# colmap/pycolmap

Measured on AMD Instinct MI355X. Metric: descriptor-pair distances/sec (exhaustive SIFT match: dot + top-2 + ratio + cross-check), higher is better.
Workload: dtype u8 descriptors, int8 MFMA / int32 accumulate; 1 GPU; 500 images x 4096 descriptors, exhaustive match + ratio test + cross-check (BASELINE.json configs[1] at N=1); pairs_total=124750, pairs_per_rank=124750, kernel=auto, matches_rank0=1865611

## Files before the change

### pycolmap_amd/csrc/match_mfma.hip

```cpp
#include <cstdlib>

#include "amc_internal.h"
#include "scan_accept.h"

namespace amc {

typedef int i32x4 __attribute__((ext_vector_type(4)));
typedef __attribute__((address_space(1))) const void gvoid_t;
typedef __attribute__((address_space(3))) void lvoid_t;

constexpr int kBN = 128;
constexpr int kYS = kBN / 32;
constexpr int kUR = 128;
constexpr int kSPB = kUR / 32;
constexpr int kChunkBytes = kBN * kDim;
constexpr int kW = kSegsPerItem;
constexpr int kWGPerCU = 2;
constexpr int kXT = kSegRows / 16;
constexpr int kKeyShift = 7, kKeyCarried = 127;

constexpr int kNB = 4;
constexpr int kOffRs = 0;
constexpr int kOffQ = kOffRs + kNB * kBN * 4;
constexpr int kOffB = kOffQ + 16;
constexpr int kLdsBytes = kOffB + kNB * kChunkBytes;
static_assert(kRowPad % kBN == 0, "a chunk divides the row padding: every chunk that holds a row lies inside the padded image");
static_assert(kUR == 128 && kSPB == 4 && kBN == kUR, "a lane quarter's rows of a block are one 32-row tile; the loop body is one block, which is one chunk");
static_assert(kRowPad % kSegRows == 0 && kSegRows % 32 == 0, "segments tile the padded rows");
static_assert((kNB & (kNB - 1)) == 0, "the ring position is taken modulo kNB with a mask");
static_assert(kWGPerCU * (kLdsBytes + 16) <= 160 * 1024, "LDS of one CU holds two workgroups (and their copy-part slots)");
static_assert(kW == 4, "one wave of a workgroup per SIMD");
static_assert(sizeof(SegDesc) == 64, "a descriptor is 16 dwords: one per lane of a quarter wave");

enum : int { kDXprep = 0, kDXrs = 2, kDOut = 4, kDList = 6, kDYprep = 8, kDYrs = 10, kDCnt = 12, kDAccword = 13,
             kDYrows = 14 };

__device__ __forceinline__ void mfma_first(i32x4& d, const i32x4& a, const i32x4& b, const i32x4& c) {
    asm volatile("v_mfma_i32_16x16x64_i8 %0, %1, %2, %3" : "=&v"(d) : "v"(a), "v"(b), "v"(c));
}
__device__ __forceinline__ void mfma_acc(i32x4& d, const i32x4& a, const i32x4& b) {
    asm volatile("v_mfma_i32_16x16x64_i8 %0, %1, %2, %0" : "+v"(d) : "v"(a), "v"(b));
}

struct YFrag {
    i32x4 f[2][2];
    i32x4 ci[2];
};

#ifdef AMC_SCAN_STAMPS
constexpr int kStampMaxWG = 1024;
__device__ uint32_t g_scan_stamps[2 * kStampMaxWG * kSegsPerItem * 8];
#define AMC_STAMP() ((uint32_t)__builtin_amdgcn_s_memtime())
#endif

__device__ __noinline__ __attribute__((used)) void copy_part(const uint4* __restrict__ src, uint4* __restrict__ dst,
                                                             unsigned long long b, unsigned long long e, int tid,
                                                             int nthreads) {
    __builtin_assume(tid >= 0 && tid < 1024 && nthreads >= 256 && nthreads <= 512);
    unsigned long long i = b + (unsigned long long)tid;
    const unsigned long long st = (unsigned long long)nthreads;
    for (; i + 3 * st < e; i += 4 * st) {
        const uint4 v0 = src[i], v1 = src[i + st], v2 = src[i + 2 * st], v3 = src[i + 3 * st];
        dst[i] = v0; dst[i + st] = v1; dst[i + 2 * st] = v2; dst[i + 3 * st] = v3;
    }
    for (; i < e; i += st) dst[i] = src[i];
}

template <int MODE>
__global__ __launch_bounds__(64 * kW) __attribute__((amdgpu_waves_per_eu(kWGPerCU, kWGPerCU)))
void match_mfma_kernel(const SegDesc* __restrict__ segs, const uint32_t* __restrict__ nitems_p,
                       uint32_t* __restrict__ queue_head, uint32_t* __restrict__ accmask,
                       const ScanAccept* __restrict__ accept, CopyJob job, uint32_t* __restrict__ copy_head) {
    static_assert(kChunkBytes / 1024 == kW * kYS, "a chunk splits into 1 KiB DMA pieces, one per wave and step");
    static_assert(kBN * 4 == 512, "a chunk's rs128 block is half a wave's DMA");
    __shared__ __attribute__((aligned(16))) char smem[kLdsBytes];

    const int tid = threadIdx.x;
    const int lane = tid & 63;
    const int wid = __builtin_amdgcn_readfirstlane(tid >> 6);
    const int l15 = lane & 15, lq = lane >> 4;
    volatile uint32_t* s_q = reinterpret_cast<volatile uint32_t*>(smem + kOffQ);
    if constexpr (MODE == 0) {
        if (job.parts) {
            __shared__ uint32_t s_part;
            if (tid == 0) s_part = atomicAdd(copy_head, 1u);
            __syncthreads();
            const uint32_t part = s_part;
            if (part < job.parts)
                copy_part(static_cast<const uint4*>(job.src), static_cast<uint4*>(job.dst), job.n16 * part / job.parts,
                          job.n16 * (part + 1) / job.parts, tid, 64 * kW);
        }
    }
    const uint32_t nitems = *nitems_p;
    const ScanAccept sa = *accept;

    auto load_desc = [&](uint32_t q) -> int {
        int v = 0;
        if (q < nitems && lane < 16) v = reinterpret_cast<const int*>(segs + (size_t)q * kSegsPerItem + wid)[lane];
        return v;
    };
    auto dword = [&](int dv, int f) -> int { return __builtin_amdgcn_readlane(dv, f); };
    auto dptr = [&](int dv, int f) -> const char* {
        const uint64_t lo = (uint32_t)__builtin_amdgcn_readlane(dv, f);
        const uint64_t hi = (uint32_t)__builtin_amdgcn_readlane(dv, f + 1);
        return reinterpret_cast<const char*>(lo | (hi << 32));
    };

    constexpr int kPW = kChunkBytes / 1024 / kW;
    auto stage_piece = [&](const char* yprep, int c, int buf, int ps) __attribute__((always_inline)) {
        const int piece = ps * kW + wid;
        __builtin_amdgcn_global_load_lds((gvoid_t*)(yprep + (size_t)c * kChunkBytes + piece * 1024 + lane * 16),
                                         (lvoid_t*)(smem + kOffB + buf * kChunkBytes + piece * 1024), 16, 0, 0);
    };
    auto stage_rs = [&](const char* yrs, int c, int buf) __attribute__((always_inline)) {
        if (wid == 0 && lane < kBN / 4)
            __builtin_amdgcn_global_load_lds((gvoid_t*)(yrs + (size_t)c * kBN * 4 + lane * 16),
                                             (lvoid_t*)(smem + kOffRs + buf * kBN * 4), 16, 0, 0);
    };
    auto stage = [&](const char* yprep, const char* yrs, int c, int buf) __attribute__((always_inline)) {
#pragma unroll
        for (int ps = 0; ps < kPW; ++ps) stage_piece(yprep, c, buf, ps);
        stage_rs(yrs, c, buf);
    };
    auto stage_head = [&](int dv) __attribute__((always_inline)) {
        const char* yprep = dptr(dv, kDYprep);
        const char* yrs = dptr(dv, kDYrs);
        const int yrows = dword(dv, kDYrows);
        stage(yprep, yrs, 0, 0);
#pragma unroll
        for (int c = 1; c < kNB - 1; ++c)
            if (yrows > c * kBN) stage(yprep, yrs, c, c);
    };

    const int yrow_lane = (kUR / 4) * (l15 >> 2) + (l15 & 3);
    const int ysw_lane = arena_swizzle(yrow_lane);
    const int yoff0 = kOffB + yrow_lane * kDim + ((lq ^ ysw_lane) * 16);
    const int yoff1 = kOffB + yrow_lane * kDim + (((4 + lq) ^ ysw_lane) * 16);
    const int coff = kOffRs + (kUR / 4) * lq * 4;
    auto load_y_part = [&](YFrag& y, int buf, int ys, int part) __attribute__((always_inline)) {
        const int ub = (ys / kSPB) * kUR, sp = ys % kSPB;
        if (part < 2) {
            const int so = buf * kBN * 4 + (ub + 8 * sp) * 4;
            y.ci[part] = *reinterpret_cast<const i32x4*>(smem + (coff + so) + 16 * part);
        } else {
            const int tt = (part - 2) >> 1, s = (part - 2) & 1;
            const int so = buf * kChunkBytes + (ub + 8 * sp) * kDim;
            y.f[tt][s] = *reinterpret_cast<const i32x4*>(smem + ((s ? yoff1 : yoff0) + so) + tt * 4 * kDim);
        }
    };
    auto load_y = [&](YFrag& y, int buf, int ys) __attribute__((always_inline)) {
#pragma unroll
        for (int part = 0; part < 6; ++part) load_y_part(y, buf, ys, part);
    };

    i32x4 xf[kXT][2];
    int best[kXT], sec[kXT], btile[kXT], xterm[kXT], part[kXT];
    auto load_x = [&](int dv) __attribute__((always_inline)) {
        const int cnt = dword(dv, kDCnt);
        const char* xprep = dptr(dv, kDXprep);
        const int* xrs = reinterpret_cast<const int*>(dptr(dv, kDXrs));
#pragma unroll
        for (int xt = 0; xt < kXT; ++xt) {
            const int kl = xt * 16 + l15;
            int row;
            if (MODE == 0) {
                row = kl;
            } else {
                const uint32_t* list = reinterpret_cast<const uint32_t*>(dptr(dv, kDList));
                row = cnt > 0 ? (int)list[min(kl, cnt - 1)] : 0;
            }
            const char* rp = xprep + (size_t)row * kDim;
            const int sw = arena_swizzle(row);
#pragma unroll
            for (int s = 0; s < 2; ++s) xf[xt][s] = *reinterpret_cast<const i32x4*>(rp + (((4 * s + lq) ^ sw) * 16));
            xterm[xt] = xrs[row] - (1 << 21);
            best[xt] = ((-xterm[xt]) << kKeyShift) | kKeyCarried;
            sec[xt] = best[xt];
            btile[xt] = -1;
        }
    };

#ifdef AMC_SCAN_STAMPS
    uint32_t st_a = 0, st_first = 0, st_end = 0, st_sum[5] = {0, 0, 0, 0, 0};
    bool st_prev = false, st_prev_active = false;
    uint32_t* const st_slot = g_scan_stamps + ((size_t)(MODE * kStampMaxWG + min((int)blockIdx.x, kStampMaxWG - 1)) * kW + wid) * 8;
#endif
    if (tid == 0) *s_q = atomicAdd(queue_head, 1u);
    __syncthreads();
    uint32_t q = *s_q;
    int dv = load_desc(q);
    if (q < nitems) {
        stage_head(dv);
        if (dword(dv, kDCnt) > 0) load_x(dv);
    }
    __syncthreads();

    while (q < nitems) {
        const char* yprep = dptr(dv, kDYprep);
        const char* yrs = dptr(dv, kDYrs);
        const int nchunks = (dword(dv, kDYrows) + kBN - 1) / kBN;
        const bool active = dword(dv, kDCnt) > 0;
        if (tid == 0) *s_q = atomicAdd(queue_head, 1u);

        i32x4 acc[2][2];
        auto insert = [&](int xt, int code) __attribute__((always_inline)) {
            asm volatile(
                "v_lshl_or_b32 %2, %2, 7, %3\n\t"
                "v_med3_i32 %1, %0, %1, %2\n\t"
                "v_max_i32 %0, %0, %2"
                : "+v"(best[xt]), "+v"(sec[xt]), "+v"(part[xt])
                : "s"(code));
        };
        auto flush = [&](int sb) __attribute__((always_inline)) {
#pragma unroll
            for (int xt = 0; xt < kXT; ++xt) {
                const int c = best[xt] & 127;
                btile[xt] = c != kKeyCarried ? sb * 64 + (126 - c) : btile[xt];
                best[xt] |= kKeyCarried;
            }
        };
        auto phase = [&](i32x4 (&an)[2], const YFrag& y, int xtn, const i32x4 (&ac)[2], int xtc, int sp, int gb)
                         __attribute__((always_inline)) {
            mfma_first(an[0], y.f[0][0], xf[xtn][0], y.ci[0]);
            mfma_first(an[1], y.f[1][0], xf[xtn][0], y.ci[1]);
            __builtin_amdgcn_sched_barrier(0);
            if (xtc == 0 ? sp == 0 : sp == kSPB - 1) {
                insert((xtc + kXT - 1) % kXT, 126 - ((xtc == 0 ? gb - 1 : gb) & 63));
                if (xtc == 0 && gb != 0 && (gb & 63) == 0) flush((gb >> 6) - 1);
                __builtin_amdgcn_sched_barrier(0);
            }
            mfma_acc(an[0], y.f[0][1], xf[xtn][1]);
            mfma_acc(an[1], y.f[1][1], xf[xtn][1]);
            __builtin_amdgcn_sched_barrier(0);
            int t0, t1;
            if (sp == 0)
                asm volatile(
                    "v_max3_i32 %0, %3, %4, %5\n\t"
                    "v_max3_i32 %1, %6, %7, %8\n\t"
                    "v_max3_i32 %0, %0, %9, %10\n\t"
                    "v_max_i32 %2, %0, %1"
                    : "=&v"(t0), "=&v"(t1), "=&v"(part[xtc])
                    : "v"(ac[0][0]), "v"(ac[0][1]), "v"(ac[0][2]), "v"(ac[0][3]), "v"(ac[1][0]), "v"(ac[1][1]),
                      "v"(ac[1][2]), "v"(ac[1][3]));
            else
                asm volatile(
                    "v_max3_i32 %0, %3, %4, %5\n\t"
                    "v_max3_i32 %1, %6, %7, %8\n\t"
                    "v_max3_i32 %0, %0, %9, %10\n\t"
                    "v_max3_i32 %2, %0, %1, %2"
                    : "=&v"(t0), "=&v"(t1), "+v"(part[xtc])
                    : "v"(ac[0][0]), "v"(ac[0][1]), "v"(ac[0][2]), "v"(ac[0][3]), "v"(ac[1][0]), "v"(ac[1][1]),
                      "v"(ac[1][2]), "v"(ac[1][3]));
            __builtin_amdgcn_sched_barrier(0);
        };

        YFrag y0, y1;
        asm volatile("s_waitcnt vmcnt(0)" ::: "memory");
        __syncthreads();
        const uint32_t qn = *s_q;
        const int dvn = load_desc(qn);
#ifdef AMC_SCAN_STAMPS
        {
            const uint32_t now = AMC_STAMP();
            if (st_prev) {
                st_sum[0] += st_a;
                st_sum[1] += now - st_end;
                st_sum[2] += now - st_first;
                st_sum[3] += 1;
                st_sum[4] += st_prev_active ? 1 : 0;
                if (lane == 0) {
#pragma unroll
                    for (int k = 0; k < 5; ++k) st_slot[k] = st_sum[k];
                }
            }
            st_a = 0;
            st_first = now;
        }
#endif
        if (active) {
            load_y(y0, 0, 0);
            mfma_first(acc[0][0], y0.f[0][0], xf[0][0], y0.ci[0]);
            mfma_first(acc[0][1], y0.f[1][0], xf[0][0], y0.ci[1]);
            mfma_acc(acc[0][0], y0.f[0][1], xf[0][1]);
            mfma_acc(acc[0][1], y0.f[1][1], xf[0][1]);
            part[kXT - 1] = -(1 << 24);
            __builtin_amdgcn_sched_barrier(0);
        }
        auto step = [&](YFrag& yc, YFrag& yn, int c, int cb, int nb, int ys) __attribute__((always_inline)) {
            const int sp = ys;
            const bool lastt = ys == kYS - 1;
            const bool cross = lastt && (c + 1 < nchunks);
            const bool fetch = c + kNB - 1 < nchunks;
            static_assert(kPW == kYS, "one DMA piece per wave and step");
            if (fetch) {
                const int fb = (cb + kNB - 1) & (kNB - 1);
                stage_piece(yprep, c + kNB - 1, fb, ys);
                if (ys == 0) stage_rs(yrs, c + kNB - 1, fb);
            }
            if (cross) {
#ifdef AMC_SCAN_STAMPS
                const uint32_t st_t = AMC_STAMP();
#endif
                static_assert(kNB == 4, "the counted waits below are written out for three chunks ahead");
                if (fetch) {
                    if (wid == 0) asm volatile("s_waitcnt vmcnt(%0)" ::"n"(2 * kPW + 2) : "memory");
                    else asm volatile("s_waitcnt vmcnt(%0)" ::"n"(2 * kPW) : "memory");
                } else if (c + 2 < nchunks) {
                    if (wid == 0) asm volatile("s_waitcnt vmcnt(%0)" ::"n"(kPW + 1) : "memory");
                    else asm volatile("s_waitcnt vmcnt(%0)" ::"n"(kPW) : "memory");
                } else {
                    asm volatile("s_waitcnt vmcnt(0)" ::: "memory");
                }
                asm volatile("s_barrier" ::: "memory");
#ifdef AMC_SCAN_STAMPS
                st_a += AMC_STAMP() - st_t;
#endif
            }
            if (active) {
                const int nbuf = cross ? nb : cb;
                const int nys = lastt ? (cross ? 0 : ys) : ys + 1;
                const int gb = c;
#pragma unroll
                for (int xt = 0; xt < kXT; ++xt) {
                    if (xt + 1 < kXT)
                        phase(acc[(xt + 1) & 1], yc, xt + 1, acc[xt & 1], xt, sp, gb);
                    else
                        phase(acc[0], yn, 0, acc[xt & 1], xt, sp, gb);
                    if (xt < 6) {
                        load_y_part(yn, nbuf, nys, xt);
                        __builtin_amdgcn_sched_barrier(0);
                    }
                }
            }
        };
#pragma unroll 1
        for (int c = 0; c < nchunks; ++c) {
            const int cb = c & (kNB - 1), nb = (c + 1) & (kNB - 1);
            step(y0, y1, c, cb, nb, 0);
            step(y1, y0, c, cb, nb, 1);
            step(y0, y1, c, cb, nb, 2);
            step(y1, y0, c, cb, nb, 3);
        }
        if (active) {
            const int lastb = nchunks - 1;
            insert(kXT - 1, 126 - (lastb & 63));
            flush(lastb >> 6);
#pragma unroll
            for (int xt = 0; xt < kXT; ++xt) {
                best[xt] >>= kKeyShift;
                sec[xt] >>= kKeyShift;
            }
        }
        __syncthreads();
#ifdef AMC_SCAN_STAMPS
        st_end = AMC_STAMP();
        st_prev = true;
        st_prev_active = active;
#endif

        int eb[kXT], es[kXT], et[kXT], ex[kXT];
#pragma unroll
        for (int xt = 0; xt < kXT; ++xt) {
            asm volatile("v_mov_b32 %0, %1" : "=v"(eb[xt]) : "v"(best[xt]));
            asm volatile("v_mov_b32 %0, %1" : "=v"(es[xt]) : "v"(sec[xt]));
            asm volatile("v_mov_b32 %0, %1" : "=v"(et[xt]) : "v"(btile[xt]));
            ex[xt] = xterm[xt];
        }
        if (qn < nitems) {
            stage_head(dvn);
            if (dword(dvn, kDCnt) > 0) load_x(dvn);
        }
        if (active) {
            const int cnt = dword(dv, kDCnt);
            uint32_t bits_lo = 0;
#pragma unroll
            for (int xt = 0; xt < kXT; ++xt) {
                const int kl = xt * 16 + l15;
                int b = eb[xt], s = es[xt], t = et[xt] < 0 ? -1 : et[xt] * kSPB + lq;
#pragma unroll
                for (int m = 16; m <= 32; m <<= 1) {
                    const int ob = __shfl_xor(b, m);
                    const int os = __shfl_xor(s, m);
                    const int ot = __shfl_xor(t, m);
                    const bool ow = (ob > b) || (ob == b && (unsigned)ot < (unsigned)t);
                    s = max(max(s, os), ow ? b : ob);
                    t = ow ? ot : t;
                    b = ow ? ob : b;
                }
                bool acc_bit = false;
                const bool live = lq == 0 && kl < cnt;
                Top2 o;
                o.best_v = (uint32_t)(b + ex[xt]);
                o.best_idx = o.best_v ? (uint32_t)t : 0xFFFFFFFFu;
                o.second_v = (uint32_t)(s + ex[xt]);
                o.pad = 0;
                if (MODE == 0) acc_bit = live && scan_may_accept(sa, o.best_v, o.second_v);
                const uint32_t bits = MODE == 0 ? (uint32_t)__ballot(acc_bit) : 0u;
                if (live && (MODE == 1 || bits != 0)) {
                    Top2* out = reinterpret_cast<Top2*>(const_cast<char*>(dptr(dv, kDOut)));
                    int row = kl;
                    if (MODE == 1) row = (int)reinterpret_cast<const uint32_t*>(dptr(dv, kDList))[kl];
                    out[row] = o;
                }
                if (MODE == 0) {
                    if (xt & 1) {
                        const uint32_t word = bits_lo | (bits << 16);
                        if (lane == 0 && word != 0) accmask[(uint32_t)dword(dv, kDAccword) + (xt >> 1)] = word;
                    } else {
                        bits_lo = bits;
                    }
                }
            }
        }
#ifdef AMC_SCAN_STAMPS
        if (qn >= nitems && lane == 0) {
            st_slot[5] = st_a;
            st_slot[6] = AMC_STAMP() - st_first;
            st_slot[7] = 1;
        }
#endif
        q = qn;
        dv = dvn;
    }
}

__device__ __forceinline__ uint32_t pair_segments(int mode, const ImageDev* imgs, const PairDev& p, uint32_t pi,
                                                  const uint32_t* cand_cnt, uint32_t* nrows_out) {
    const uint32_t nx = mode == 0 ? imgs[p.slot1].rows : cand_cnt[pi];
    const uint32_t ny = imgs[mode == 0 ? p.slot2 : p.slot1].rows;
    *nrows_out = nx;
    return ny ? (nx + kSegRows - 1) / kSegRows : 0u;
}

__global__ __launch_bounds__(256) void seg_count_kernel(int mode, const ImageDev* __restrict__ imgs,
                                                        const PairDev* __restrict__ pairs,
                                                        const uint32_t* __restrict__ order,
                                                        const uint32_t* __restrict__ grp_start,
                                                        const uint32_t* __restrict__ cand_cnt,
                                                        uint32_t* __restrict__ seg_base, uint32_t* __restrict__ grp_segs) {
    __shared__ uint32_t wsum[4];
    const uint32_t g = blockIdx.x, tid = threadIdx.x, lane = tid & 63, wid = tid >> 6;
    const uint32_t i0 = grp_start[g], i1 = grp_start[g + 1];
    uint32_t running = 0;
    for (uint32_t base = i0; base < i1; base += 256) {
        const uint32_t i = base + tid;
        uint32_t s = 0, nr;
        if (i < i1) {
            const uint32_t pi = order[i];
            s = pair_segments(mode, imgs, pairs[pi], pi, cand_cnt, &nr);
        }
        uint32_t inc = s;
#pragma unroll
        for (int m = 1; m < 64; m <<= 1) {
            const uint32_t o = __shfl_up(inc, m);
            if (lane >= (uint32_t)m) inc += o;
        }
        if (lane == 63) wsum[wid] = inc;
        __syncthreads();
        uint32_t wbase = 0, total = 0;
        for (uint32_t k = 0; k < 4; ++k) {
            if (k < wid) wbase += wsum[k];
            total += wsum[k];
        }
        if (i < i1) seg_base[i] = running + wbase + inc - s;
        running += total;
        __syncthreads();
    }
    if (tid == 0) grp_segs[g] = running;
}

__global__ __launch_bounds__(1024) void seg_scan_kernel(const uint32_t* __restrict__ grp_segs, uint32_t ngroups,
                                                        uint32_t* __restrict__ grp_item_base,
                                                        uint32_t* __restrict__ nitems_out) {
    __shared__ uint32_t wsum[16];
    const uint32_t tid = threadIdx.x, lane = tid & 63, wid = tid >> 6;
    uint32_t running = 0;
    for (uint32_t base = 0; base < ngroups; base += 1024) {
        const uint32_t g = base + tid;
        const uint32_t s = g < ngroups ? (grp_segs[g] + kSegsPerItem - 1) / kSegsPerItem : 0u;
        uint32_t inc = s;
#pragma unroll
        for (int m = 1; m < 64; m <<= 1) {
            const uint32_t o = __shfl_up(inc, m);
            if (lane >= (uint32_t)m) inc += o;
        }
        if (lane == 63) wsum[wid] = inc;
        __syncthreads();
        uint32_t wbase = 0, total = 0;
        for (uint32_t k = 0; k < 16; ++k) {
            if (k < wid) wbase += wsum[k];
            total += wsum[k];
        }
        if (g < ngroups) grp_item_base[g] = running + wbase + inc - s;
        running += total;
        __syncthreads();
    }
    if (tid == 0) *nitems_out = running;
}

constexpr uint32_t kFillY = 8;
__global__ __launch_bounds__(256) void seg_fill_kernel(int mode, const ImageDev* __restrict__ imgs,
                                                       const PairDev* __restrict__ pairs,
                                                       const uint32_t* __restrict__ order,
                                                       const uint32_t* __restrict__ grp_start,
                                                       const uint32_t* __restrict__ cand_cnt,
                                                       const uint32_t* __restrict__ candbuf,
                                                       const uint32_t* __restrict__ seg_base,
                                                       const uint32_t* __restrict__ grp_segs,
                                                       const uint32_t* __restrict__ grp_item_base,
                                                       Top2* __restrict__ outbuf, SegDesc* __restrict__ segs) {
    const uint32_t g = blockIdx.x, tid = threadIdx.x, lane = tid & 63, wid = blockIdx.y * 4 + (tid >> 6);
    const uint32_t i0 = grp_start[g], i1 = grp_start[g + 1];
    if (i0 >= i1) return;
    const uint32_t total = grp_segs[g];
    if (total == 0) return;
    SegDesc* gs = segs + (size_t)grp_item_base[g] * kSegsPerItem;
    const PairDev p0 = pairs[order[i0]];
    const ImageDev Y = imgs[mode == 0 ? p0.slot2 : p0.slot1];
    for (uint32_t i = i0 + wid; i < i1; i += 4 * kFillY) {
        const uint32_t pi = order[i];
        const PairDev p = pairs[pi];
        uint32_t nx;
        const uint32_t ns = pair_segments(mode, imgs, p, pi, cand_cnt, &nx);
        const ImageDev X = imgs[mode == 0 ? p.slot1 : p.slot2];
        const uint32_t sb = seg_base[i];
        for (uint32_t k = lane; k < ns; k += 64) {
            const uint32_t row0 = k * kSegRows;
            SegDesc d;
            d.yprep = Y.prep;
            d.yrs = Y.rs128;
            d.yrows = Y.rows;
            d.cnt = min(nx - row0, (uint32_t)kSegRows);
            d.pad_ = 0;
            if (mode == 0) {
                d.xprep = X.prep + (size_t)row0 * kDim;
                d.xrs = X.rs128 + row0;
                d.out = outbuf + p.row_off + row0;
                d.list = nullptr;
                d.accword = (uint32_t)((p.row_off + row0) >> 5);
            } else {
                d.xprep = X.prep;
                d.xrs = X.rs128;
                d.out = outbuf + p.col_off;
                d.list = candbuf + p.col_off + row0;
                d.accword = 0;
            }
            gs[sb + k] = d;
        }
    }
    const uint32_t padded = (total + kSegsPerItem - 1) / kSegsPerItem * kSegsPerItem;
    if (blockIdx.y == 0 && tid < padded - total) {
        SegDesc d;
        d.xprep = Y.prep;
        d.xrs = Y.rs128;
        d.out = nullptr;
        d.list = nullptr;
        d.yprep = Y.prep;
        d.yrs = Y.rs128;
        d.cnt = 0;
        d.accword = 0;
        d.yrows = Y.rows;
        d.pad_ = 0;
        gs[total + tid] = d;
    }
}

hipError_t launch_build_segments(int mode, const ImageDev* imgs, const PairDev* pairs, const uint32_t* order,
                                 const uint32_t* grp_start, uint32_t ngroups, const uint32_t* cand_cnt,
                                 const uint32_t* candbuf, Top2* outbuf, uint32_t* seg_base, uint32_t* grp_segs,
                                 uint32_t* grp_item_base, SegDesc* segs, uint32_t* nitems_dev, hipStream_t s) {
    if (ngroups == 0) return memset_async(nitems_dev, 0, sizeof(uint32_t), s);
    hipLaunchKernelGGL(seg_count_kernel, dim3(ngroups), dim3(256), 0, s, mode, imgs, pairs, order, grp_start,
                       cand_cnt, seg_base, grp_segs);
    hipLaunchKernelGGL(seg_scan_kernel, dim3(1), dim3(1024), 0, s, grp_segs, ngroups, grp_item_base, nitems_dev);
    hipLaunchKernelGGL(seg_fill_kernel, dim3(ngroups, kFillY), dim3(256), 0, s, mode, imgs, pairs, order, grp_start,
                       cand_cnt, candbuf, seg_base, grp_segs, grp_item_base, outbuf, segs);
    return hipGetLastError();
}

hipError_t launch_match_mfma(int mode, const SegDesc* segs, const uint32_t* nitems_dev, uint32_t max_items,
                             uint32_t* queue_head, uint32_t* accmask, const ScanAccept* accept_dev, hipStream_t s,
                             const CopyJob& job_in, uint32_t* copy_head) {
    if (max_items == 0) return hipSuccess;
    CopyJob job = (mode == 0 && copy_head) ? job_in : CopyJob();
    hipError_t e = job.parts ? memset_async(copy_head, 0, sizeof(uint32_t), s) : hipSuccess;
    if (e != hipSuccess) return e;
    int dev = 0, cus = 256;
    if ((e = hipGetDevice(&dev)) != hipSuccess) return e;
    if ((e = hipDeviceGetAttribute(&cus, hipDeviceAttributeMultiprocessorCount, dev)) != hipSuccess) return e;
    static const hipError_t occupancy = [] {
        int n0 = 0, n1 = 0;
        hipError_t oe = hipOccupancyMaxActiveBlocksPerMultiprocessor(&n0, match_mfma_kernel<0>, 64 * kW, 0);
        if (oe == hipSuccess) oe = hipOccupancyMaxActiveBlocksPerMultiprocessor(&n1, match_mfma_kernel<1>, 64 * kW, 0);
        if (oe != hipSuccess) return oe;
        return n0 >= kWGPerCU && n1 >= kWGPerCU ? hipSuccess : hipErrorLaunchOutOfResources;
    }();
    if (occupancy != hipSuccess) return occupancy;
    int wgs = kWGPerCU * cus;
    static const int grid_cap = [] {
        const char* e = std::getenv("AMC_SCAN_GRID");
        return e ? std::atoi(e) : 0;
    }();
    if (grid_cap > 0 && grid_cap < wgs) wgs = grid_cap;
    const uint32_t grid = max_items < (uint32_t)wgs ? max_items : (uint32_t)wgs;
    if (job.parts > grid) job.parts = grid;
    if ((e = memset_async(queue_head, 0, sizeof(uint32_t), s)) != hipSuccess) return e;
    if (mode == 0)
        hipLaunchKernelGGL((match_mfma_kernel<0>), dim3(grid), dim3(64 * kW), 0, s, segs, nitems_dev, queue_head,
                           accmask, accept_dev, job, copy_head);
    else
        hipLaunchKernelGGL((match_mfma_kernel<1>), dim3(grid), dim3(64 * kW), 0, s, segs, nitems_dev, queue_head,
                           accmask, accept_dev, job, copy_head);
    return hipGetLastError();
}

}
```

Before: 13580 billion distances/s.

## Split chunk loop into steady/drain phases with incrementally advanced LDS offsets

Splits the per-chunk scan loop into a steady-state loop, which always prefetches three chunks ahead, and a drain loop, which does not prefetch. This removes the per-step fetch/cross branching. LDS read bases for the Y fragments and rs values are now advanced by inline-asm adds at each chunk crossing instead of being recomputed from the buffer index. Global-load lane offsets are pinned in a register, inactive workgroups get their own loop that only issues the DMA and barriers, and the copy-part slot moves into the existing LDS queue area to drop a separate shared variable. The aim is to cut scalar and vector address arithmetic and control flow in the inner loop. The cost is more code, and the offset rewind and barrier counts must match between active and inactive waves.

```diff
diff --git a/pycolmap_amd/csrc/match_mfma.hip b/pycolmap_amd/csrc/match_mfma.hip
--- a/pycolmap_amd/csrc/match_mfma.hip
+++ b/pycolmap_amd/csrc/match_mfma.hip
@@ -28,7 +28,7 @@
 static_assert(kUR == 128 && kSPB == 4 && kBN == kUR, "a lane quarter's rows of a block are one 32-row tile; the loop body is one block, which is one chunk");
 static_assert(kRowPad % kSegRows == 0 && kSegRows % 32 == 0, "segments tile the padded rows");
 static_assert((kNB & (kNB - 1)) == 0, "the ring position is taken modulo kNB with a mask");
-static_assert(kWGPerCU * (kLdsBytes + 16) <= 160 * 1024, "LDS of one CU holds two workgroups (and their copy-part slots)");
+static_assert(kWGPerCU * kLdsBytes <= 160 * 1024, "LDS of one CU holds two workgroups");
 static_assert(kW == 4, "one wave of a workgroup per SIMD");
 static_assert(sizeof(SegDesc) == 64, "a descriptor is 16 dwords: one per lane of a quarter wave");
 
@@ -82,10 +82,10 @@
     volatile uint32_t* s_q = reinterpret_cast<volatile uint32_t*>(smem + kOffQ);
     if constexpr (MODE == 0) {
         if (job.parts) {
-            __shared__ uint32_t s_part;
-            if (tid == 0) s_part = atomicAdd(copy_head, 1u);
+            volatile uint32_t* s_part = reinterpret_cast<volatile uint32_t*>(smem + kOffQ + 4);
+            if (tid == 0) *s_part = atomicAdd(copy_head, 1u);
             __syncthreads();
-            const uint32_t part = s_part;
+            const uint32_t part = *s_part;
             if (part < job.parts)
                 copy_part(static_cast<const uint4*>(job.src), static_cast<uint4*>(job.dst), job.n16 * part / job.parts,
                           job.n16 * (part + 1) / job.parts, tid, 64 * kW);
@@ -107,15 +107,22 @@
     };
 
     constexpr int kPW = kChunkBytes / 1024 / kW;
+    uint32_t lane16 = (uint32_t)lane * 16u;
+    auto lane_off = [&]() __attribute__((always_inline)) -> uint32_t {
+        asm volatile("" : "+v"(lane16));
+        return lane16;
+    };
     auto stage_piece = [&](const char* yprep, int c, int buf, int ps) __attribute__((always_inline)) {
         const int piece = ps * kW + wid;
-        __builtin_amdgcn_global_load_lds((gvoid_t*)(yprep + (size_t)c * kChunkBytes + piece * 1024 + lane * 16),
+        const char* src = yprep + ((size_t)c * kChunkBytes + piece * 1024);
+        __builtin_amdgcn_global_load_lds((gvoid_t*)(src + lane_off()),
                                          (lvoid_t*)(smem + kOffB + buf * kChunkBytes + piece * 1024), 16, 0, 0);
     };
     auto stage_rs = [&](const char* yrs, int c, int buf) __attribute__((always_inline)) {
+        const char* src = yrs + (size_t)c * kBN * 4;
         if (wid == 0 && lane < kBN / 4)
-            __builtin_amdgcn_global_load_lds((gvoid_t*)(yrs + (size_t)c * kBN * 4 + lane * 16),
-                                             (lvoid_t*)(smem + kOffRs + buf * kBN * 4), 16, 0, 0);
+            __builtin_amdgcn_global_load_lds((gvoid_t*)(src + lane_off()), (lvoid_t*)(smem + kOffRs + buf * kBN * 4), 16, 0,
+                                             0);
     };
     auto stage = [&](const char* yprep, const char* yrs, int c, int buf) __attribute__((always_inline)) {
 #pragma unroll
@@ -134,23 +141,25 @@
 
     const int yrow_lane = (kUR / 4) * (l15 >> 2) + (l15 & 3);
     const int ysw_lane = arena_swizzle(yrow_lane);
-    const int yoff0 = kOffB + yrow_lane * kDim + ((lq ^ ysw_lane) * 16);
-    const int yoff1 = kOffB + yrow_lane * kDim + (((4 + lq) ^ ysw_lane) * 16);
-    const int coff = kOffRs + (kUR / 4) * lq * 4;
-    auto load_y_part = [&](YFrag& y, int buf, int ys, int part) __attribute__((always_inline)) {
-        const int ub = (ys / kSPB) * kUR, sp = ys % kSPB;
+    int yb0 = kOffB + yrow_lane * kDim + ((lq ^ ysw_lane) * 16);
+    int yb1 = kOffB + yrow_lane * kDim + (((4 + lq) ^ ysw_lane) * 16);
+    int cbs = kOffRs + (kUR / 4) * lq * 4;
+    auto load_y_part = [&](YFrag& y, int ys, int part) __attribute__((always_inline)) {
         if (part < 2) {
-            const int so = buf * kBN * 4 + (ub + 8 * sp) * 4;
-            y.ci[part] = *reinterpret_cast<const i32x4*>(smem + (coff + so) + 16 * part);
+            y.ci[part] = *reinterpret_cast<const i32x4*>(smem + cbs + (8 * ys * 4 + 16 * part));
         } else {
             const int tt = (part - 2) >> 1, s = (part - 2) & 1;
-            const int so = buf * kChunkBytes + (ub + 8 * sp) * kDim;
-            y.f[tt][s] = *reinterpret_cast<const i32x4*>(smem + ((s ? yoff1 : yoff0) + so) + tt * 4 * kDim);
-        }
-    };
-    auto load_y = [&](YFrag& y, int buf, int ys) __attribute__((always_inline)) {
-#pragma unroll
-        for (int part = 0; part < 6; ++part) load_y_part(y, buf, ys, part);
+            y.f[tt][s] = *reinterpret_cast<const i32x4*>(smem + (s ? yb1 : yb0) + (8 * ys + tt * 4) * kDim);
+        }
+    };
+    auto load_y = [&](YFrag& y, int ys) __attribute__((always_inline)) {
+#pragma unroll
+        for (int part = 0; part < 6; ++part) load_y_part(y, ys, part);
+    };
+    auto advance = [&](int cb) __attribute__((always_inline)) {
+        const int k = cb == kNB - 1 ? -(kNB - 1) : 1;
+        asm volatile("v_add_u32 %0, %3, %0\n\tv_add_u32 %1, %3, %1\n\tv_add_u32 %2, %4, %2"
+                     : "+v"(yb0), "+v"(yb1), "+v"(cbs) : "s"(k * kChunkBytes), "s"(k * kBN * 4));
     };
 
     i32x4 xf[kXT][2];
@@ -277,71 +286,77 @@
             st_first = now;
         }
 #endif
+        static_assert(kPW == kYS, "one DMA piece per wave and step");
+        static_assert(kNB == 4, "the counted waits below are written out for three chunks ahead");
+        auto crossing = [&](bool steady, int rem) __attribute__((always_inline)) {
+#ifdef AMC_SCAN_STAMPS
+            const uint32_t st_t = AMC_STAMP();
+#endif
+            if (steady) {
+                if (wid == 0) asm volatile("s_waitcnt vmcnt(%0)" ::"n"(2 * kPW + 2) : "memory");
+                else asm volatile("s_waitcnt vmcnt(%0)" ::"n"(2 * kPW) : "memory");
+            } else if (rem >= 2) {
+                if (wid == 0) asm volatile("s_waitcnt vmcnt(%0)" ::"n"(kPW + 1) : "memory");
+                else asm volatile("s_waitcnt vmcnt(%0)" ::"n"(kPW) : "memory");
+            } else {
+                asm volatile("s_waitcnt vmcnt(0)" ::: "memory");
+            }
+            asm volatile("s_barrier" ::: "memory");
+#ifdef AMC_SCAN_STAMPS
+            st_a += AMC_STAMP() - st_t;
+#endif
+        };
+        auto fetch = [&](int c, int cb, int ys) __attribute__((always_inline)) {
+            const int fb = (cb + kNB - 1) & (kNB - 1);
+            stage_piece(yprep, c + kNB - 1, fb, ys);
+            if (ys == 0) stage_rs(yrs, c + kNB - 1, fb);
+        };
+        int c = 0, cb = 0;
         if (active) {
-            load_y(y0, 0, 0);
+            load_y(y0, 0);
             mfma_first(acc[0][0], y0.f[0][0], xf[0][0], y0.ci[0]);
             mfma_first(acc[0][1], y0.f[1][0], xf[0][0], y0.ci[1]);
             mfma_acc(acc[0][0], y0.f[0][1], xf[0][1]);
             mfma_acc(acc[0][1], y0.f[1][1], xf[0][1]);
             part[kXT - 1] = -(1 << 24);
             __builtin_amdgcn_sched_barrier(0);
-        }
-        auto step = [&](YFrag& yc, YFrag& yn, int c, int cb, int nb, int ys) __attribute__((always_inline)) {
-            const int sp = ys;
-            const bool lastt = ys == kYS - 1;
-            const bool cross = lastt && (c + 1 < nchunks);
-            const bool fetch = c + kNB - 1 < nchunks;
-            static_assert(kPW == kYS, "one DMA piece per wave and step");
-            if (fetch) {
-                const int fb = (cb + kNB - 1) & (kNB - 1);
-                stage_piece(yprep, c + kNB - 1, fb, ys);
-                if (ys == 0) stage_rs(yrs, c + kNB - 1, fb);
-            }
-            if (cross) {
-#ifdef AMC_SCAN_STAMPS
-                const uint32_t st_t = AMC_STAMP();
-#endif
-                static_assert(kNB == 4, "the counted waits below are written out for three chunks ahead");
-                if (fetch) {
-                    if (wid == 0) asm volatile("s_waitcnt vmcnt(%0)" ::"n"(2 * kPW + 2) : "memory");
-                    else asm volatile("s_waitcnt vmcnt(%0)" ::"n"(2 * kPW) : "memory");
-                } else if (c + 2 < nchunks) {
-                    if (wid == 0) asm volatile("s_waitcnt vmcnt(%0)" ::"n"(kPW + 1) : "memory");
-                    else asm volatile("s_waitcnt vmcnt(%0)" ::"n"(kPW) : "memory");
-                } else {
-                    asm volatile("s_waitcnt vmcnt(0)" ::: "memory");
+            auto step = [&](YFrag& yc, YFrag& yn, int ys, bool steady) __attribute__((always_inline)) {
+                if (steady) fetch(c, cb, ys);
+                if (ys == kYS - 1) {
+                    const int rem = nchunks - 1 - c;
+                    if (steady || rem >= 1) crossing(steady, rem);
+                    advance(cb);
                 }
-                asm volatile("s_barrier" ::: "memory");
-#ifdef AMC_SCAN_STAMPS
-                st_a += AMC_STAMP() - st_t;
-#endif
-            }
-            if (active) {
-                const int nbuf = cross ? nb : cb;
-                const int nys = lastt ? (cross ? 0 : ys) : ys + 1;
-                const int gb = c;
+                const int nys = ys == kYS - 1 ? 0 : ys + 1;
 #pragma unroll
                 for (int xt = 0; xt < kXT; ++xt) {
                     if (xt + 1 < kXT)
-                        phase(acc[(xt + 1) & 1], yc, xt + 1, acc[xt & 1], xt, sp, gb);
+                        phase(acc[(xt + 1) & 1], yc, xt + 1, acc[xt & 1], xt, ys, c);
                     else
-                        phase(acc[0], yn, 0, acc[xt & 1], xt, sp, gb);
+                        phase(acc[0], yn, 0, acc[xt & 1], xt, ys, c);
                     if (xt < 6) {
-                        load_y_part(yn, nbuf, nys, xt);
+                        load_y_part(yn, nys, xt);
                         __builtin_amdgcn_sched_barrier(0);
                     }
                 }
-            }
-        };
+            };
 #pragma unroll 1
-        for (int c = 0; c < nchunks; ++c) {
-            const int cb = c & (kNB - 1), nb = (c + 1) & (kNB - 1);
-            step(y0, y1, c, cb, nb, 0);
-            step(y1, y0, c, cb, nb, 1);
-            step(y0, y1, c, cb, nb, 2);
-            step(y1, y0, c, cb, nb, 3);
-        }
-        if (active) {
+            for (; c + kNB - 1 < nchunks; ++c, cb = (cb + 1) & (kNB - 1)) {
+                step(y0, y1, 0, true);
+                step(y1, y0, 1, true);
+                step(y0, y1, 2, true);
+                step(y1, y0, 3, true);
+            }
+#pragma unroll 1
+            for (; c < nchunks; ++c, cb = (cb + 1) & (kNB - 1)) {
+                step(y0, y1, 0, false);
+                step(y1, y0, 1, false);
+                step(y0, y1, 2, false);
+                step(y1, y0, 3, false);
+            }
+            yb0 -= cb * kChunkBytes;
+            yb1 -= cb * kChunkBytes;
+            cbs -= cb * kBN * 4;
             const int lastb = nchunks - 1;
             insert(kXT - 1, 126 - (lastb & 63));
             flush(lastb >> 6);
@@ -350,6 +365,15 @@
                 best[xt] >>= kKeyShift;
                 sec[xt] >>= kKeyShift;
             }
+        } else {
+#pragma unroll 1
+            for (; c + kNB - 1 < nchunks; ++c, cb = (cb + 1) & (kNB - 1)) {
+#pragma unroll
+                for (int ys = 0; ys < kYS; ++ys) fetch(c, cb, ys);
+                crossing(true, kNB - 1);
+            }
+#pragma unroll 1
+            for (; c + 1 < nchunks; ++c) crossing(false, nchunks - 1 - c);
         }
         __syncthreads();
 #ifdef AMC_SCAN_STAMPS
```

After: 14150 billion distances/s (median of 6 runs). 4.2% higher.
